# dronefreak/CABiNet

Hardware: AMD Instinct MI355X
Metric: 1024x1024 images/sec fwd+bwd (CABiNet-MobileNetV3-Large) (higher is better)
Workload: dtype f32; 1 GPU; BASELINE configs[2]: CABiNet-MobileNetV3-Large, 8x3x1024x1024 synthetic 8-class per GPU, fwd + 2x OhemCE + bwd + grad all-reduce + SGD step, HIP CAB/FFM kernels, fp32, random-init (model seed 0, gamma=0.5); per_gpu_batch=8, global_batch=8, n_classes=8, parallelism=dp1, miopen_find_mode=FAST

## Files before the change

### cabinet_amd/_lib.py

```python

from __future__ import annotations

import ctypes
import os
import threading

_PKG_DIR = os.path.dirname(os.path.abspath(__file__))
LIB_PATH = os.path.join(_PKG_DIR, "libcabinet_hip.so")
ABI_VERSION = 8

_c_float_p = ctypes.c_void_p
_INT, _FLT, _SZ, _PTR = ctypes.c_int, ctypes.c_float, ctypes.c_size_t, ctypes.c_void_p

SIGNATURES = {
    "cabinet_abi_version": (_INT, []),
    "cabinet_last_error": (ctypes.c_char_p, []),
    "cabinet_cab_attn_supported": (_INT, [_INT] * 2),
    "cabinet_cab_attn_precision_supported": (_INT, [_INT] * 3),
    "cabinet_cab_attn_fwd_workspace_bytes": (_SZ, [_INT] * 5),
    "cabinet_cab_attn_fwd": (_INT, [_PTR, _PTR, _PTR, _FLT, _INT, _INT, _INT, _INT, _INT, _PTR, _PTR, _PTR, _SZ, _PTR]),
    "cabinet_cab_attn_proj_supported": (_INT, [_INT] * 5),
    "cabinet_cab_attn_proj_fwd": (_INT, [_PTR] * 4 + [_FLT] + [_INT] * 5 + [_PTR] * 3 + [_PTR]),
    "cabinet_cab_attn_bwd_workspace_bytes": (_SZ, [_INT] * 4),
    "cabinet_cab_attn_bwd": (_INT, [_PTR] * 6 + [_FLT] + [_INT] * 4 + [_PTR] * 3 + [_PTR, _SZ, _PTR]),
# ... 22 lines not shown
    "cabinet_ohem_up_w_bwd_sel": (_INT, [_PTR] * 3 + [_INT] * 6 + [_PTR, _INT, _FLT] + [_PTR] + [_PTR, _SZ] + [_PTR, _PTR]),
    "cabinet_ohem_up_pair_w_bwd_sel": (_INT, [_PTR] * 4 + [_INT] * 6 + [_PTR, _INT, _FLT] + [_PTR] + [_PTR, _SZ] + [_PTR, _PTR, _PTR]),
    "cabinet_focal_up_supported": (_INT, [_INT] * 5 + [_FLT]),
    "cabinet_focal_up_fwd": (_INT, [_PTR] * 3 + [_INT] * 6 + [_FLT, _FLT, _INT] + [_PTR] * 3 + [_PTR, _PTR, _PTR]),
    "cabinet_focal_stats": (_INT, [_PTR, _PTR, _INT, _INT, _PTR, _PTR]),
    "cabinet_focal_up_bwd_workspace_bytes": (_SZ, [_INT] * 7),
    "cabinet_focal_up_bwd": (_INT, [_PTR] * 4 + [_INT] * 6 + [_FLT, _FLT, _INT, _FLT] + [_PTR] + [_PTR, _SZ] + [_PTR, _PTR, _PTR]),
    "cabinet_cab_qkv_supported": (_INT, [_INT] * 7 + [_PTR]),
    "cabinet_cab_qkv_padded_bins": (_INT, [_INT, _PTR]),
    "cabinet_cab_qkv_fwd_workspace_bytes": (_SZ, [_INT] * 7 + [_PTR]),
    "cabinet_cab_qkv_fwd": (_INT, [_PTR] * 14 + [_INT] * 7 + [_PTR] + [_INT, _FLT, _FLT] + [_PTR] * 10
                            + [_PTR, _SZ, _PTR]),
    "cabinet_cab_qkv_bwd_workspace_bytes": (_SZ, [_INT] * 7 + [_PTR]),
    "cabinet_cab_qkv_bwd": (_INT, [_PTR] * 20 + [_INT] * 7 + [_PTR] + [_INT] + [_PTR] * 9 + [_PTR, _SZ, _PTR]),
    "cabinet_conv1x1_fwd_workspace_bytes": (_SZ, [_INT] * 2),
    "cabinet_conv1x1_fwd": (_INT, [_PTR] * 2 + [_INT] * 4 + [_PTR] + [_PTR, _SZ, _PTR]),
    "cabinet_conv1x1_bias_supported": (_INT, [_INT] * 4),
    "cabinet_conv1x1_bias_fwd": (_INT, [_PTR] * 3 + [_INT] * 4 + [_PTR] + [_PTR, _SZ, _PTR]),
    "cabinet_channel_sum": (_INT, [_PTR] + [_INT] * 3 + [_PTR] + [_PTR]),
    "cabinet_conv1x1_bwd_workspace_bytes": (_SZ, [_INT] * 4),
    "cabinet_conv1x1_bwd": (_INT, [_PTR] * 3 + [_INT] * 4 + [_PTR] * 2 + [_PTR, _SZ, _PTR]),
    "cabinet_bn_act_workspace_bytes": (_SZ, [_INT] * 3),
    "cabinet_bn_act_fwd": (_INT, [_PTR] * 6 + [_INT] * 5 + [_FLT, _FLT] + [_PTR] * 3 + [_PTR, _SZ, _PTR]),
    "cabinet_bn_act_bwd": (_INT, [_PTR] * 6 + [_INT] * 5 + [_PTR] * 3 + [_PTR, _SZ, _PTR]),
    "cabinet_bn_cls_supported": (_INT, [_INT] * 3),
    "cabinet_bn_cls_table_floats": (_INT, [_INT] * 2),
    "cabinet_bn_cls_fwd_workspace_bytes": (_SZ, [_INT] * 3),
    "cabinet_bn_cls_fwd": (_INT, [_PTR] * 8 + [_INT] * 6 + [_FLT, _FLT] + [_PTR] * 2 + [_PTR, _SZ, _PTR]),
    "cabinet_bn_cls_bwd_workspace_bytes": (_SZ, [_INT] * 4),
    "cabinet_bn_cls_bwd": (_INT, [_PTR] * 3 + [_INT] * 6 + [_PTR] * 5 + [_PTR, _SZ, _PTR]),
    "cabinet_gate_act_fwd": (_INT, [_PTR] * 2 + [_INT] * 4 + [_PTR] + [_PTR]),
    "cabinet_gate_act_bwd_workspace_bytes": (_SZ, [_INT] * 3),
    "cabinet_gate_act_bwd": (_INT, [_PTR] * 3 + [_INT] * 4 + [_PTR] * 2 + [_PTR, _SZ, _PTR]),
    "cabinet_bn_dwconv_fwd_workspace_bytes": (_SZ, [_INT] * 4),
    "cabinet_bn_dwconv_fwd": (_INT, [_PTR] * 6 + [_INT] * 8 + [_FLT, _FLT] + [_PTR] * 3 + [_PTR, _SZ, _PTR]),
    "cabinet_bn_dwconv_bwd_workspace_bytes": (_SZ, [_INT] * 6),
    "cabinet_bn_dwconv_bwd": (_INT, [_PTR] * 7 + [_INT] * 8 + [_PTR] * 4 + [_PTR, _SZ, _PTR]),
    "cabinet_stem_conv_fwd": (_INT, [_PTR] * 2 + [_INT] * 3 + [_PTR] + [_PTR]),
    "cabinet_stem_conv_wrw_workspace_bytes": (_SZ, [_INT] * 3),
    "cabinet_stem_conv_wrw": (_INT, [_PTR] * 2 + [_INT] * 3 + [_PTR] + [_PTR, _SZ, _PTR]),
    "cabinet_stem_conv_bn_bwd_workspace_bytes": (_SZ, [_INT] * 3),
    "cabinet_stem_conv_bn_bwd": (_INT, [_PTR] * 7 + [_INT] * 4 + [_PTR] * 3 + [_PTR, _SZ, _PTR]),
    "cabinet_pwconv_supported": (_INT, [_INT] * 3),
    "cabinet_pwconv_fwd": (_INT, [_PTR] * 2 + [_INT] * 4 + [_PTR] + [_PTR]),
    "cabinet_pwconv_bwd_workspace_bytes": (_SZ, [_INT] * 4),
    "cabinet_pwconv_bwd": (_INT, [_PTR] * 3 + [_INT] * 4 + [_PTR] * 2 + [_PTR, _SZ, _PTR]),
    "cabinet_pwconv_wide_supported": (_INT, [_INT] * 3),
    "cabinet_pwconv_wide_wgrad_workspace_bytes": (_SZ, [_INT] * 4),
    "cabinet_pwconv_wide_wgrad": (_INT, [_PTR] * 2 + [_INT] * 4 + [_PTR] + [_PTR, _SZ, _PTR]),
    "cabinet_conv3x3s2_supported": (_INT, [_INT] * 2),
    "cabinet_conv3x3s2_wgrad_workspace_bytes": (_SZ, [_INT] * 5),
    "cabinet_conv3x3s2_wgrad": (_INT, [_PTR] * 2 + [_INT] * 5 + [_PTR] + [_PTR, _SZ, _PTR]),
    "cabinet_conv3x3s2_dgrad": (_INT, [_PTR] * 2 + [_INT] * 5 + [_PTR] + [_PTR]),
    "cabinet_bn_act_fwd_part": (_INT, [_PTR] * 7 + [_INT] * 6 + [_FLT, _FLT] + [_PTR] * 3 + [_PTR]),
    "cabinet_conv3x3_supported": (_INT, [_INT] * 3),
    "cabinet_conv3x3_tile_blocks": (_INT, [_INT] * 3),
    "cabinet_conv3x3_fwd_workspace_bytes": (_SZ, [_INT] * 6),
    "cabinet_conv3x3_fwd": (_INT, [_PTR] * 3 + [_INT] * 6 + [_PTR] * 2 + [_PTR, _SZ, _PTR]),
    "cabinet_conv3x3_bwd_workspace_bytes": (_SZ, [_INT] * 6),
    "cabinet_conv3x3_bwd": (_INT, [_PTR] * 4 + [_INT] * 6 + [_PTR] * 3 + [_PTR, _SZ, _PTR]),
    "cabinet_dwconv_supported": (_INT, [_INT] * 2),
    "cabinet_dwconv_fwd": (_INT, [_PTR] * 2 + [_INT] * 6 + [_PTR] + [_PTR]),
    "cabinet_dwconv_bwd_workspace_bytes": (_SZ, [_INT] * 6),
    "cabinet_dwconv_bwd": (_INT, [_PTR] * 3 + [_INT] * 6 + [_PTR] * 2 + [_PTR, _SZ, _PTR]),
    "cabinet_cab_local_supported": (_INT, [_INT] * 4),
    "cabinet_cab_local_fwd_workspace_bytes": (_SZ, [_INT] * 4),
    "cabinet_cab_local_bwd_workspace_bytes": (_SZ, [_INT] * 4),
    "cabinet_cab_local_fwd": (_INT, [_PTR] * 3 + [_PTR] * 5 + [_INT] * 5 + [_FLT, _FLT] + [_PTR] * 3 + [_PTR, _SZ, _PTR]),
    "cabinet_cab_local_bwd": (_INT, [_PTR] * 4 + [_PTR] * 3 + [_PTR] * 2 + [_INT] * 5 + [_PTR] * 3 + [_PTR] * 3 + [_PTR, _SZ, _PTR]),
    "cabinet_eval_chip_accum_supported": (_INT, [_INT] * 6),
    "cabinet_eval_chip_accum": (_INT, [_PTR] * 2 + [_INT] * 6 + [_PTR] + [_INT] * 4 + [_PTR] * 2 + [_PTR]),
    "cabinet_eval_scale_merge": (_INT, [_PTR] + [_INT] * 8 + [_PTR] + [_INT] * 2 + [_PTR]),
    "cabinet_eval_argmax_hist": (_INT, [_PTR] * 2 + [_INT] * 5 + [_PTR] * 2 + [_PTR]),
    "cabinet_predict_up_argmax_supported": (_INT, [_INT] * 5),
    "cabinet_predict_up_argmax": (_INT, [_PTR] + [_INT] * 6 + [_PTR] + [_PTR]),
    "cabinet_predict_argmax": (_INT, [_PTR] + [_INT] * 4 + [_PTR] + [_PTR]),
    "cabinet_predict_render": (_INT, [_PTR] * 3 + [_INT] + [_PTR] * 2 + [_FLT] + [_INT] * 3 + [_PTR] * 3 + [_PTR]),
    "cabinet_se_act_bwd_workspace_bytes": (_SZ, [_INT] * 3),
    "cabinet_se_act_bwd_reduce": (_INT, [_PTR] * 8 + [_INT] * 4 + [_PTR] * 2 + [_PTR, _SZ, _PTR]),
    "cabinet_se_act_bwd_coef": (_INT, [_PTR] * 3 + [_INT] * 4 + [_PTR] * 4 + [_PTR]),
    "cabinet_se_act_bwd_dx": (_INT, [_PTR] * 9 + [_INT] * 4 + [_PTR] + [_PTR]),
    "cabinet_sgd_tail_workspace_bytes": (_SZ, [_INT]),
    "cabinet_sgd_tail_state_bytes": (_SZ, [_INT]),
    "cabinet_sgd_tail_step": (_INT, [_PTR, _INT, _PTR, _INT, _PTR, _PTR, _SZ, _INT, _PTR, _SZ, _PTR]),
    "cabinet_grad_accum_state_bytes": (_SZ, []),
    "cabinet_grad_accum": (_INT, [_PTR, _INT, _PTR, _INT, _PTR, _SZ, _INT, _PTR]),
    "cabinet_grad_accum_reset": (_INT, [_PTR, _SZ, _PTR]),
    "cabinet_augment_supported": (_INT, [_INT] * 7),
    "cabinet_augment_workspace_bytes": (_SZ, [_INT] * 3),
    "cabinet_augment_batch": (_INT, [_PTR] + [_INT] * 3 + [_PTR, ctypes.c_ulonglong] + [_PTR] * 5 + [_PTR, _SZ, _PTR]),
    "cabinet_augment_warp_supported": (_INT, [_INT] * 4 + [ctypes.c_double] * 2),
    "cabinet_augment_warp_batch": (_INT, [_PTR] + [_INT] * 3 + [_PTR]),
    "cabinet_augment_resize_batch": (_INT, [_PTR] + [_INT] * 3 + [_PTR]),
}

_lock = threading.Lock()
_lib = None


def _preload_hip_runtime():
    import sys

    cands = []
    if "torch" in sys.modules:
        cands.append(os.path.join(os.path.dirname(sys.modules["torch"].__file__), "lib", "libamdhip64.so"))
    cands += ["libamdhip64.so.7", "/opt/rocm/lib/libamdhip64.so.7"]
# ... 44 lines not shown
```

### cabinet_amd/csrc/capi.hip

```cpp
#include "../../include/cabinet_hip.h"

#include <stdarg.h>
#include <stdint.h>
#include <stdio.h>

#include "blocks.hpp"
#include "cab_local.hpp"
#include "cab_qkv.hpp"
#include "common.hpp"

namespace cabinet {
int attn_fwd_kvsplit(int B, int n);
bool attn_shape_supported(int Kc, int Vc);
hipError_t attn_fwd_dispatch(const float* q, const float* k, const float* v, float scale, int B, int Kc,
                             int Vc, int n, float* ctx, float* lse, float* part_ctx, float* part_lse,
                             int kvsplit, hipStream_t stream);
bool attn_fwd_proj_supported(int B, int Kc, int Vc, int Co, int n);
hipError_t attn_fwd_proj_dispatch(const float* q, const float* k, const float* v, const float* w_out, float scale, int B, int Kc,
                                  int Vc, int Co, int n, float* ctx, float* glob, float* lse, hipStream_t stream);
bool attn_bf16_supported(int Kc, int Vc);
size_t attn_bf16_pack_bytes(int B, int Kc, int Vc, int n, int precision);
hipError_t attn_fwd_bf16_dispatch(const float* q, const float* k, const float* v, float scale, int B, int Kc, int Vc, int n,
                                  float* ctx, float* lse, float* part_ctx, float* part_lse, int kvsplit, void* pack, int precision,
                                  hipStream_t stream);
// ... 49 lines not shown
hipError_t se_act_bwd_coef_run(const float* sums, const float* gate, const float* ds, int B, int C, int P, int training,
                               float* dweight, float* dbias, float* coef, float* ds_p, hipStream_t stream);
hipError_t se_act_bwd_dx_run(const float* dy, const float* z, const float* mean, const float* invstd, const float* weight,
                             const float* bias, const float* gate, const float* ds_p, const float* coef, int B, int C, int P,
                             int act, float* dz, hipStream_t stream);
size_t gate_act_workspace(int rows, int P);
hipError_t gate_act_fwd_run(const float* x, const float* gate, int rows, int P, int act, float* y, hipStream_t stream);
hipError_t gate_act_bwd_run(const float* dy, const float* x, const float* gate, int rows, int P, int act, float* dx,
                            float* dgate, void* ws, hipStream_t stream);
bool bn_cls_supported(int C, int K, int P);
int bn_cls_table_floats(int C, int K);
size_t bn_cls_fwd_workspace(int B, int C, int P);
size_t bn_cls_bwd_workspace(int B, int C, int K, int P);
hipError_t bn_cls_fwd_run(const float* z, const float* conv_part, const float* bn_w, const float* bn_b, float* run_mean, float* run_var,
                          const float* w_cls, const float* bias, int B, int C, int K, int H, int W, int training, float momentum,
                          float eps, float* y, float* tab, void* ws, hipStream_t stream);
hipError_t bn_cls_bwd_run(const float* dy, const float* z, const float* tab, int B, int C, int K, int H, int W, int training, float* dz,
                          float* dbn_w, float* dbn_b, float* dw_cls, float* dbias, void* ws, hipStream_t stream);
bool dwconv_supported(int K, int S);
size_t dwconv_bwd_workspace(int B, int C, int H, int W, int K);
hipError_t dwconv_fwd_run(const float* x, const float* w, int B, int C, int H, int W, int K, int S, float* y,
                          hipStream_t stream);
hipError_t dwconv_bwd_run(const float* dy, const float* x, const float* w, int B, int C, int H, int W, int K, int S,
                          float* dx, float* dw, void* ws, hipStream_t stream);
size_t bn_dwconv_fwd_workspace(int B, int C, int H, int W);
size_t bn_dwconv_bwd_workspace(int B, int C, int H, int W, int K);
hipError_t bn_dwconv_fwd_run(const float* z, const float* bn_w, const float* bn_b, float* run_mean, float* run_var,
                             const float* w, int B, int C, int H, int W, int K, int S, int act, int training,
                             float momentum, float eps, float* y, float* save_mean, float* save_invstd, void* ws,
                             hipStream_t stream);
hipError_t bn_dwconv_bwd_run(const float* dy, const float* z, const float* bn_w, const float* bn_b,
                             const float* save_mean, const float* save_invstd, const float* w, int B, int C, int H,
                             int W, int K, int S, int act, int training, float* dz, float* dbn_w, float* dbn_b,
                             float* dw, void* ws, hipStream_t stream);
size_t stem_conv_wrw_workspace(int B, int H, int W);
hipError_t stem_conv_fwd_run(const float* x, const float* w, int B, int H, int W, float* y, hipStream_t stream);
size_t stem_conv_bn_bwd_workspace(int B, int H, int W);
hipError_t stem_conv_bn_bwd_run(const float* g, const float* z, const float* x, const float* bn_weight, const float* bn_bias,
                                const float* save_mean, const float* save_invstd, int B, int H, int W, int training, float* dw,
                                float* dbn_weight, float* dbn_bias, void* ws, hipStream_t stream);
hipError_t stem_conv_wrw_run(const float* dy, const float* x, int B, int H, int W, float* dw, void* ws,
                             hipStream_t stream);
bool pwconv_wide_supported(int Ci, int Co, int P);
size_t pwconv_wide_wgrad_workspace(int B, int Ci, int Co, int P);
hipError_t pwconv_wide_wgrad_run(const float* dy, const float* x, int B, int Ci, int Co, int P, float* dw, void* ws,
                                 hipStream_t stream);
bool conv3x3s2_supported(int Ci, int Co);
long long conv3x3s2_wgrad_slabs(int B, int Ci, int H, int W);
size_t conv3x3s2_wgrad_workspace(int B, int Ci, int H, int W);
hipError_t conv3x3s2_wgrad_run(const float* dy, const float* x, int B, int Ci, int H, int W, float* dw, void* ws,
                               hipStream_t stream);
long long conv3x3s2_dgrad_workgroups(int B, int H, int W);
hipError_t conv3x3s2_dgrad_run(const float* dy, const float* w, int B, int H, int W, float* dx, hipStream_t stream);
bool pwconv_supported(int Ci, int Co, int P);
size_t pwconv_bwd_workspace(int B, int Ci, int Co, int P);
hipError_t pwconv_fwd_run(const float* x, const float* w, int B, int Ci, int Co, int P, float* y, hipStream_t stream);
hipError_t pwconv_bwd_run(const float* dy, const float* x, const float* w, int B, int Ci, int Co, int P, float* dx,
                          float* dw, void* ws, hipStream_t stream);
int ohem_blocks(int B, int H, int W);
hipError_t ohem_up_fwd_run(int nh, const float* const* low, const long long* labels, int B, int C, int Hl, int Wl, int H, int W,
                           float thresh, int ignore_lb, float* const* loss_px, float* const* blk_sum, int* const* blk_cnt,
                           const float* const* class_weight, hipStream_t stream, const float* focal_gamma = nullptr);
hipError_t focal_stats_run(const float* blk_sum, const int* blk_cnt, int nheads, int nblk, double* stats, hipStream_t stream);
hipError_t ohem_stats_run(const float* blk_sum, const int* blk_cnt, int nheads, int nblk, double* stats, hipStream_t stream);
size_t ohem_up_bwd_workspace(int B, int C, int H, int Wl);
bool ohem_up_supported(int C, int Wl, int W);
hipError_t ohem_up_bwd_run(int nh, const float* const* low, const long long* labels, const float* const* loss_px, int B, int C,
                           int Hl, int Wl, int H, int W, float thresh, int ignore_lb, float coef, float* dlow, void* ws,
                           const float* const* cw, const double* dsel, hipStream_t stream, const float* focal_gamma = nullptr);
size_t ohem_select_workspace(int nheads);
hipError_t ohem_select_run(int nheads, const float* const* loss_px, const long long* labels, const double* stats, long long P, int C,
                           float thresh, const int* n_min, int ignore_lb, const float* const* cw, double* sel, void* ws,
                           hipStream_t stream);
struct WinoShape {
    int B, C0, C1, K, H, W;
};
bool conv3x3_supported(int C0, int C1, int K);
bool conv3x3_shape_ok(const WinoShape& s);
int conv3x3_tile_blocks(int B, int H, int W);
size_t conv3x3_fwd_workspace(const WinoShape& s);
size_t conv3x3_bwd_workspace(const WinoShape& s);
hipError_t conv3x3_fwd_run(const WinoShape& s, const float* x0, const float* x1, const float* w, float* y, float* stat_part, void* ws,
                           hipStream_t stream);
hipError_t conv3x3_bwd_run(const WinoShape& s, const float* dy, const float* x0, const float* x1, const float* w, float* dx0,
                           float* dx1, float* dw, void* ws, hipStream_t stream);
int eval_chip_threads(int C, int wl, int cw, int nsrc);
hipError_t eval_chip_accum_run(const float* a, const float* b, int N, int C, int hl, int wl, int ch, int cw, float* dst, int FH,
                               int FW, int y0, int x0, const float* rcp_y, const float* rcp_x, hipStream_t stream);
hipError_t eval_scale_merge_run(const float* prob, int N, int C, int FH, int FW, int hst, int hed, int wst, int wed, float* total,
                                int H, int W, hipStream_t stream);
hipError_t eval_argmax_hist_run(const float* total, const long long* labels, int N, int C, int H, int W, int ignore_lb, long long* hist,
                                unsigned char* pred, hipStream_t stream);
int predict_up_threads(int C, int wl, int W);
hipError_t predict_up_argmax_run(const float* a, int N, int C, int hl, int wl, int H, int W, unsigned char* labels, hipStream_t stream);
hipError_t predict_argmax_run(const float* total, int N, int C, int H, int W, unsigned char* labels, hipStream_t stream);
hipError_t predict_render_run(const unsigned char* labels, const float* image, const unsigned char* palette, int n_colors,
                              const float* mean, const float* std, float alpha, int N, int H, int W, unsigned char* pred,
                              unsigned char* inp, unsigned char* ovl, hipStream_t stream);
hipError_t augment_warp_run(const void* descs, int N, int max_oh, int max_ow, hipStream_t stream);
hipError_t augment_resize_run(const void* descs, int N, int max_oh, int max_ow, hipStream_t stream);
size_t augment_workspace(int N, int th, int tw);
hipError_t augment_run(const void* samples, int N, int th, int tw, const float* noise, unsigned long long seed, const float* mean,
                       const float* std, float* out_image, long long* out_label, unsigned char* out_u8, void* workspace,
                       hipStream_t stream);
size_t sgd_tail_workspace(int n_chunks);
size_t sgd_tail_state(int n_entries);
// ... 1115 lines not shown
        return fail(CABINET_ERR_UNSUPPORTED, "pwconv_wide_wgrad: B=%d, P=%d: more than 2^30 pixel chunks", B, P);
    if (!cabinet::pwconv_wide_supported(Ci, Co, P))
        return fail(CABINET_ERR_UNSUPPORTED, "pwconv_wide_wgrad: Ci=%d, Co=%d, P=%d (multiples of 8, <= 4096, P <= 2^21, max(Ci, Co) * P <= 2^28)",
                    Ci, Co, P);
    if (!dy || !x || !dw) return fail(CABINET_ERR_INVALID_ARG, "pwconv_wide_wgrad: null tensor pointer");
    const size_t need = cabinet::pwconv_wide_wgrad_workspace(B, Ci, Co, P);
    if (!workspace || workspace_bytes < need)
        return fail(CABINET_ERR_WORKSPACE, "pwconv_wide_wgrad: workspace %zu < %zu bytes", workspace_bytes, need);
    return hip_status(cabinet::pwconv_wide_wgrad_run(dy, x, B, Ci, Co, P, dw, workspace, static_cast<hipStream_t>(stream)),
                      "pwconv_wide_wgrad launch");
}

static bool conv3x3s2_size_ok(int B, int Ci, int H, int W) {
    return cabinet::conv3x3s2_wgrad_slabs(B, Ci, H, W) <= (1ll << 30);
}

int cabinet_conv3x3s2_supported(int Ci, int Co) { return cabinet::conv3x3s2_supported(Ci, Co) ? 1 : 0; }

size_t cabinet_conv3x3s2_wgrad_workspace_bytes(int B, int Ci, int Co, int H, int W) {
    if (B <= 0 || H <= 0 || W <= 0 || !cabinet::conv3x3s2_supported(Ci, Co) || !conv3x3s2_size_ok(B, Ci, H, W)) return 0;
    return cabinet::conv3x3s2_wgrad_workspace(B, Ci, H, W);
}

int cabinet_conv3x3s2_wgrad(const float* dy, const float* x, int B, int Ci, int Co, int H, int W, float* dw, void* workspace,
                            size_t workspace_bytes, cabinet_stream_t stream) {
    if (B <= 0 || Ci <= 0 || Co <= 0 || H <= 0 || W <= 0)
        return fail(CABINET_ERR_INVALID_ARG, "conv3x3s2_wgrad: non-positive dimension");
    if (!cabinet::conv3x3s2_supported(Ci, Co))
        return fail(CABINET_ERR_UNSUPPORTED, "conv3x3s2_wgrad: Ci=%d, Co=%d ((64, 64) and (3, 16) are compiled)", Ci, Co);
    if (!conv3x3s2_size_ok(B, Ci, H, W))
        return fail(CABINET_ERR_UNSUPPORTED, "conv3x3s2_wgrad: B=%d, H=%d, W=%d: grid too large", B, H, W);
    if (!dy || !x || !dw) return fail(CABINET_ERR_INVALID_ARG, "conv3x3s2_wgrad: null tensor pointer");
    const size_t need = cabinet::conv3x3s2_wgrad_workspace(B, Ci, H, W);
    if (!workspace || workspace_bytes < need)
        return fail(CABINET_ERR_WORKSPACE, "conv3x3s2_wgrad: workspace %zu < %zu bytes", workspace_bytes, need);
    return hip_status(cabinet::conv3x3s2_wgrad_run(dy, x, B, Ci, H, W, dw, workspace, static_cast<hipStream_t>(stream)),
                      "conv3x3s2_wgrad launch");
}

int cabinet_conv3x3s2_dgrad(const float* dy, const float* w, int B, int Ci, int Co, int H, int W, float* dx,
                            cabinet_stream_t stream) {
    if (B <= 0 || Ci <= 0 || Co <= 0 || H <= 0 || W <= 0)
        return fail(CABINET_ERR_INVALID_ARG, "conv3x3s2_dgrad: non-positive dimension");
    if (Ci != 64 || Co != 64)
        return fail(CABINET_ERR_UNSUPPORTED, "conv3x3s2_dgrad: Ci=%d, Co=%d ((64, 64) is compiled)", Ci, Co);
    if (cabinet::conv3x3s2_dgrad_workgroups(B, H, W) > (1ll << 30))
        return fail(CABINET_ERR_UNSUPPORTED, "conv3x3s2_dgrad: B=%d, H=%d, W=%d: grid too large", B, H, W);
    if (!dy || !w || !dx) return fail(CABINET_ERR_INVALID_ARG, "conv3x3s2_dgrad: null tensor pointer");
    if ((reinterpret_cast<size_t>(dx) & 7) != 0)
        return fail(CABINET_ERR_INVALID_ARG, "conv3x3s2_dgrad: dx must be 8-byte aligned");
    return hip_status(cabinet::conv3x3s2_dgrad_run(dy, w, B, H, W, dx, static_cast<hipStream_t>(stream)), "conv3x3s2_dgrad launch");
}

static int check_conv3x3(const cabinet::WinoShape& s, const char* who) {
    if (s.B <= 0 || s.C0 <= 0 || s.C1 < 0 || s.K <= 0 || s.H <= 0 || s.W <= 0)
        return fail(CABINET_ERR_INVALID_ARG, "%s: non-positive dimension", who);
    if (!cabinet::conv3x3_shape_ok(s))
        return fail(CABINET_ERR_UNSUPPORTED,
                    "%s: C0=%d C1=%d Co=%d H=%d W=%d (C0, C1 multiples of 16; Co, C0+C1 multiples of 64; C0 %% 64 == 0 when C1 > 0; "
                    "one image's tensors < 1 GiB)", who, s.C0, s.C1, s.K, s.H, s.W);
    return CABINET_OK;
}

int cabinet_conv3x3_supported(int C0, int C1, int Co) { return cabinet::conv3x3_supported(C0, C1, Co) ? 1 : 0; }

int cabinet_conv3x3_tile_blocks(int B, int H, int W) {
    return B > 0 && H > 0 && W > 0 ? cabinet::conv3x3_tile_blocks(B, H, W) : 0;
}

size_t cabinet_conv3x3_fwd_workspace_bytes(int B, int C0, int C1, int Co, int H, int W) {
    const cabinet::WinoShape s{B, C0, C1, Co, H, W};
    return B > 0 && H > 0 && W > 0 && cabinet::conv3x3_shape_ok(s) ? cabinet::conv3x3_fwd_workspace(s) : 0;
}

int cabinet_conv3x3_fwd(const float* x0, const float* x1, const float* w, int B, int C0, int C1, int Co, int H, int W, float* y,
                        float* bn_part, void* workspace, size_t workspace_bytes, cabinet_stream_t stream) {
    const cabinet::WinoShape s{B, C0, C1, Co, H, W};
    if (int rc = check_conv3x3(s, "conv3x3_fwd")) return rc;
    if (!x0 || !w || !y || (C1 > 0 && !x1)) return fail(CABINET_ERR_INVALID_ARG, "conv3x3_fwd: null tensor pointer");
    CABINET_REQUIRE_ALIGNED("conv3x3_fwd", x0, x1, w, y, bn_part);
    const size_t need = cabinet::conv3x3_fwd_workspace(s);
    if (!workspace || workspace_bytes < need)
        return fail(CABINET_ERR_WORKSPACE, "conv3x3_fwd: workspace %zu < %zu bytes", workspace_bytes, need);
    return hip_status(cabinet::conv3x3_fwd_run(s, x0, C1 > 0 ? x1 : nullptr, w, y, bn_part, workspace, static_cast<hipStream_t>(stream)),
                      "conv3x3_fwd launch");
}

size_t cabinet_conv3x3_bwd_workspace_bytes(int B, int C0, int C1, int Co, int H, int W) {
    const cabinet::WinoShape s{B, C0, C1, Co, H, W};
    return B > 0 && H > 0 && W > 0 && cabinet::conv3x3_shape_ok(s) ? cabinet::conv3x3_bwd_workspace(s) : 0;
}

int cabinet_conv3x3_bwd(const float* dy, const float* x0, const float* x1, const float* w, int B, int C0, int C1, int Co, int H,
                        int W, float* dx0, float* dx1, float* dw, void* workspace, size_t workspace_bytes, cabinet_stream_t stream) {
    const cabinet::WinoShape s{B, C0, C1, Co, H, W};
    if (int rc = check_conv3x3(s, "conv3x3_bwd")) return rc;
    if (!dy || !w || (dw && (!x0 || (C1 > 0 && !x1))) || (dx0 && C1 > 0 && !dx1))
        return fail(CABINET_ERR_INVALID_ARG, "conv3x3_bwd: null tensor pointer");
    CABINET_REQUIRE_ALIGNED("conv3x3_bwd", dy, x0, x1, w, dx0, dx1, dw);
    const size_t need = cabinet::conv3x3_bwd_workspace(s);
    if (!workspace || workspace_bytes < need)
        return fail(CABINET_ERR_WORKSPACE, "conv3x3_bwd: workspace %zu < %zu bytes", workspace_bytes, need);
    return hip_status(cabinet::conv3x3_bwd_run(s, dy, x0, C1 > 0 ? x1 : nullptr, w, dx0, C1 > 0 ? dx1 : nullptr, dw, workspace,
                                               static_cast<hipStream_t>(stream)),
                      "conv3x3_bwd launch");
}
// ... 209 lines not shown
```

### cabinet_amd/csrc/conv3x3_s2.hip

```cpp
#include "common.hpp"
#include "slab_sum.hpp"

namespace cabinet {

struct C3Shape {
    int B, H, W, Ho, Wo;
};

static C3Shape c3_shape(int B, int H, int W) { return C3Shape{B, H, W, (H - 1) / 2 + 1, (W - 1) / 2 + 1}; }

constexpr int CW_C = 64;
constexpr int CW_TW = 32;
constexpr int CW_IW = 2 * CW_TW + 1;
constexpr int CW_XP = 3 * CW_IW;
constexpr int CW_DLD = CW_TW + 1;
constexpr int CW_SLAB = CW_C * CW_C * 9;
constexpr int CW_TARGET_WG = 512;
constexpr int CW_MIN_ROWS = 4;

struct C3Plan {
    int tiles_x, strips, rows_per;
};

static C3Plan cw_plan(const C3Shape& s) {
// ... 236 lines not shown
        const float* bp0 = brow + s0 * CD_RP;
        const float* bp1 = brow + s1 * CD_RP;
        s0 = s1;
#pragma unroll 1
        for (int ng = 0; ng < CD_NT / 16 && n0 + 16 * ng < s.Wo; ++ng) {
            f32x4v acc[2][2];
#pragma unroll
            for (int i = 0; i < 2; ++i)
#pragma unroll
                for (int j = 0; j < 2; ++j) acc[i][j] = f32x4v{0.f, 0.f, 0.f, 0.f};
            float bv[2][8];
            auto read_half = [&](int g, float* v) {
                const int t = g / 2;
                const float* bt = (cd_shift(t / 3) ? bp1 : bp0) + 16 * ng + cd_shift(t % 3);
#pragma unroll
                for (int i = 0; i < 8; ++i) v[i] = bt[4 * (8 * (g % 2) + i) * CD_CP];
            };
            read_half(0, bv[0]);
            f32x4v p0, p1;
#pragma unroll
            for (int g = 0; g < 18; ++g) {
                const int t = g / 2, k8 = 8 * (g % 2);
                if (g + 1 < 18) read_half(g + 1, bv[(g + 1) & 1]);
                if (g % 2 == 0) p0 = p1 = f32x4v{0.f, 0.f, 0.f, 0.f};
#pragma unroll
                for (int i = 0; i < 8; i += 2) {
                    p0 = mfma16(wr[t][k8 + i], bv[g & 1][i], p0);
                    p1 = mfma16(wr[t][k8 + i + 1], bv[g & 1][i + 1], p1);
                }
                if (g % 2 == 1) acc[cd_par(t / 3)][cd_par(t % 3)] += p0 + p1;
                __builtin_amdgcn_sched_barrier(0);
            }
            const int ix = 2 * (n0 + 16 * ng + lc);
#pragma unroll
            for (int rp = 0; rp < 2; ++rp) {
                const int iy = 2 * m + rp;
                if (iy < s.H && ix < s.W) {
#pragma unroll
                    for (int r = 0; r < 4; ++r) {
                        float* p = dxb + ((size_t)r * s.H + iy) * s.W + ix;
                        if (pair_ok) {
                            *reinterpret_cast<f32x2*>(p) = f32x2{acc[rp][0][r], acc[rp][1][r]};
                        } else {
                            p[0] = acc[rp][0][r];
                            if (ix + 1 < s.W) p[1] = acc[rp][1][r];
                        }
                    }
                }
            }
        }
    }
}

bool conv3x3s2_supported(int Ci, int Co) { return (Ci == CW_C && Co == CW_C) || (Ci == CF_CI && Co == CF_CO); }

static C3Plan cd_plan(const C3Shape& s) {
    C3Plan p;
    p.tiles_x = ceil_div(s.Wo, CD_NT);
    const long per = (long)s.B * p.tiles_x;
    long strips = CW_TARGET_WG / per;
    if (strips > s.Ho) strips = s.Ho;
    if (strips < 1) strips = 1;
    p.rows_per = ceil_div(s.Ho, (int)strips);
    p.strips = ceil_div(s.Ho, p.rows_per);
    return p;
}

long long conv3x3s2_dgrad_workgroups(int B, int H, int W) {
    const C3Shape s = c3_shape(B, H, W);
    const long long per = (long long)B * ceil_div(s.Wo, CD_NT);
    if (per > (1ll << 30)) return per;
    const C3Plan p = cd_plan(s);
    return per * p.strips;
}

hipError_t conv3x3s2_dgrad_run(const float* dy, const float* w, int B, int H, int W, float* dx, hipStream_t stream) {
    const C3Shape s = c3_shape(B, H, W);
    const C3Plan p = cd_plan(s);
    hipLaunchKernelGGL(conv3x3s2_dgrad64_kernel, dim3(B * p.tiles_x * p.strips), dim3(256), 0, stream, dy, w, s, p.tiles_x,
                       p.strips, p.rows_per, dx);
    return hipGetLastError();
}

long long conv3x3s2_wgrad_slabs(int B, int Ci, int H, int W) {
    const C3Shape s = c3_shape(B, H, W);
    if (Ci == CF_CI) return (long long)B * ceil_div(s.Ho, CF_TH);
    const long long tiles_x = ceil_div(s.Wo, CW_TW);
    if ((long long)B * tiles_x > (1ll << 30)) return (long long)B * tiles_x;
    const C3Plan p = cw_plan(s);
    return (long long)B * p.tiles_x * p.strips;
}

size_t conv3x3s2_wgrad_workspace(int B, int Ci, int H, int W) {
    return align_up((size_t)conv3x3s2_wgrad_slabs(B, Ci, H, W) * (Ci == CF_CI ? CF_SLAB : CW_SLAB) * sizeof(float), 256);
}

hipError_t conv3x3s2_wgrad_run(const float* dy, const float* x, int B, int Ci, int H, int W, float* dw, void* ws,
                               hipStream_t stream) {
    const C3Shape s = c3_shape(B, H, W);
    float* slabs = static_cast<float*>(ws);
    const int nslab = (int)conv3x3s2_wgrad_slabs(B, Ci, H, W);
    if (Ci == CF_CI) {
        hipLaunchKernelGGL(conv3x3s2_wgrad_3_16_kernel, dim3(nslab), dim3(256), 0, stream, dy, x, s, ceil_div(s.Wo, CF_TW),
                           slabs);
    } else {
        const C3Plan p = cw_plan(s);
        const size_t lds = (size_t)(CW_C * CW_XP + CW_C * CW_DLD) * sizeof(float);
// ... 14 lines not shown
```

### cabinet_amd/functional.py

```python

from __future__ import annotations

import ctypes as _ct

import torch
import torch.nn.functional as F

from . import _lib


def _ptr(t):
    return t.data_ptr() if t is not None else None


def _stream_handle(device):
    return torch.cuda.current_stream(device).cuda_stream


def _workspace(nbytes, device):
    if nbytes == 0:
        return None, 0
    ws = torch.empty(nbytes, dtype=torch.uint8, device=device)
    return ws, nbytes

# ... 1626 lines not shown
                                                   _stream_handle(x.device))
            _lib.check(rc, "cabinet_pwconv_wide_wgrad")
        return dx, dw


def pwconv_wide(x, conv):
    if not x.is_cuda:
        raise RuntimeError("pwconv_wide: device tensors only")
    return _PwConvWide.apply(x, conv.weight)




CONV3X3S2_ENABLED = _os.environ.get("CABINET_CONV3X3S2", "1") != "0"


def conv3x3s2_supported(conv, x):
    if not (CONV3X3S2_ENABLED and isinstance(conv, torch.nn.Conv2d) and x.is_cuda and x.dim() == 4):
        return False
    if not (conv.kernel_size == (3, 3) and conv.stride == (2, 2) and conv.padding == (1, 1) and conv.groups == 1
            and conv.bias is None and conv.dilation == (1, 1) and conv.padding_mode == "zeros"):
        return False
    if not (torch.is_grad_enabled() and conv.weight.requires_grad) or torch.is_autocast_enabled():
        return False
    if x.dtype != torch.float32 or conv.weight.dtype != torch.float32 or x.shape[0] < 1 or x.shape[2] * x.shape[3] < 1:
        return False
    return x.shape[1] == conv.in_channels and bool(_lib.load().cabinet_conv3x3s2_supported(conv.in_channels, conv.out_channels))


def _conv3x3s2_native_wgrad(Ci, B, H):
    return Ci == 3 and B * (((H - 1) // 2 + 1 + 3) // 4) >= 1024


CONV3X3S2_WGRAD64_ENABLED = _os.environ.get("CABINET_CONV3X3S2_WGRAD64", "1") != "0"
_CW_MIN_WORKGROUPS = 256
_CW_MIN_ROWS = 4


def _conv3x3s2_wgrad64_plan(B, H, W):
    Ho, Wo = (H - 1) // 2 + 1, (W - 1) // 2 + 1
    tiles = -(-Wo // 32)
    strips = max(1, min(512 // (B * tiles), -(-Ho // 4)))
    rows_per = -(-Ho // strips)
    return B * tiles * -(-Ho // rows_per), rows_per


def _conv3x3s2_native_wgrad64(B, H, W):
    if not CONV3X3S2_WGRAD64_ENABLED:
        return False
    workgroups, rows_per = _conv3x3s2_wgrad64_plan(B, H, W)
    return workgroups >= _CW_MIN_WORKGROUPS and rows_per >= _CW_MIN_ROWS


class _Conv3x3S2(torch.autograd.Function):

    @staticmethod
    def forward(fn_ctx, x, weight):
        x = x.contiguous()
        y = F.conv2d(x, weight, None, 2, 1)
        fn_ctx.save_for_backward(x, weight)
        return y

    @staticmethod
    def backward(fn_ctx, g):
        x, w = fn_ctx.saved_tensors
        g = g.contiguous()
        lib = _lib.load()
        xc, gc = _f32c(x), _f32c(g)
        Co, Ci = w.shape[0], w.shape[1]
        B, H, W = xc.shape[0], xc.shape[2], xc.shape[3]
        cb = torch.ops.aten.convolution_backward
        dx = None
        if fn_ctx.needs_input_grad[0] and Ci == 64:
            dx = torch.empty_like(xc)
            with torch.cuda.device(x.device):
                rc = lib.cabinet_conv3x3s2_dgrad(_ptr(gc), _ptr(_f32c(w)), B, Ci, Co, H, W, _ptr(dx), _stream_handle(x.device))
            _lib.check(rc, "cabinet_conv3x3s2_dgrad")
        elif fn_ctx.needs_input_grad[0]:
            dx = cb(g, x, w, None, [2, 2], [1, 1], [1, 1], False, [0, 0], 1, [True, False, False])[0]
        dw = None
        native_dw = _conv3x3s2_native_wgrad64(B, H, W) if Ci == 64 else _conv3x3s2_native_wgrad(Ci, B, H)
        if fn_ctx.needs_input_grad[1] and native_dw:
            dw = torch.empty((Co, Ci, 3, 3), dtype=torch.float32, device=x.device)
            ws, nbytes = _workspace(lib.cabinet_conv3x3s2_wgrad_workspace_bytes(B, Ci, Co, H, W), x.device)
            with torch.cuda.device(x.device):
                rc = lib.cabinet_conv3x3s2_wgrad(_ptr(gc), _ptr(xc), B, Ci, Co, H, W, _ptr(dw), _ptr(ws), nbytes,
                                                 _stream_handle(x.device))
            _lib.check(rc, "cabinet_conv3x3s2_wgrad")
        elif fn_ctx.needs_input_grad[1]:
            dw = cb(g, x, w, None, [2, 2], [1, 1], [1, 1], False, [0, 0], 1, [False, True, False])[1]
        return dx, dw


class Conv2dS2(torch.nn.Conv2d):

    def _conv_forward(self, input, weight, bias):
        if bias is None and conv3x3s2_supported(self, input):
            return _Conv3x3S2.apply(input, weight)
        return super()._conv_forward(input, weight, bias)




def eval_chip_accum_supported(logits, chip_size, flip=False):
    if not (logits.is_cuda and logits.dim() == 4 and _lib.available()):
        return False
    _, C, hl, wl = logits.shape
    return bool(_lib.load().cabinet_eval_chip_accum_supported(C, hl, wl, int(chip_size[0]), int(chip_size[1]), int(bool(flip))))


def eval_chip_accum(dst, logits, logits_flipped, chip_size, origin, rcp_y=None, rcp_x=None):
    lib = _lib.load()
    if not (dst.is_cuda and dst.dtype == torch.float32 and dst.is_contiguous()):
        raise RuntimeError("eval_chip_accum: dst must be a dense fp32 device tensor")
    a = _f32c(logits)
    b = _f32c(logits_flipped) if logits_flipped is not None else None
    if b is not None and b.shape != a.shape:
        raise RuntimeError("eval_chip_accum: the flipped chip's logits must have the shape of the chip's")
    N, C, hl, wl = a.shape
    if dst.shape[:2] != (N, C):
        raise RuntimeError(f"eval_chip_accum: dst {tuple(dst.shape)} does not match logits {tuple(a.shape)}")
    FH, FW = dst.shape[2:]
    ry = _f32c(rcp_y) if rcp_y is not None else None
    rx = _f32c(rcp_x) if rcp_x is not None else None
    if (ry is not None and ry.numel() != FH) or (rx is not None and rx.numel() != FW):
        raise RuntimeError("eval_chip_accum: rcp_y / rcp_x must have one entry per row / column of dst")
    dev = dst.device
    with torch.cuda.device(dev):
        rc = lib.cabinet_eval_chip_accum(_ptr(a), _ptr(b), N, C, hl, wl, int(chip_size[0]), int(chip_size[1]), _ptr(dst), FH, FW,
                                         int(origin[0]), int(origin[1]), _ptr(ry), _ptr(rx), _stream_handle(dev))
    _lib.check(rc, "cabinet_eval_chip_accum")
    return dst


def eval_scale_merge_supported(total):
    return bool(total.is_cuda and total.dim() == 4 and _lib.available() and total.shape[0] * total.shape[1] <= 65535
                and total.shape[2] <= 65535)


def eval_scale_merge(total, prob, crop=None):
    lib = _lib.load()
    if not (total.is_cuda and total.dtype == torch.float32 and total.is_contiguous()):
        raise RuntimeError("eval_scale_merge: total must be a dense fp32 device tensor")
    prob = _f32c(prob)
    N, C, H, W = total.shape
    if prob.shape[:2] != (N, C):
        raise RuntimeError(f"eval_scale_merge: prob {tuple(prob.shape)} does not match total {tuple(total.shape)}")
    FH, FW = prob.shape[2:]
    hst, hed, wst, wed = crop if crop is not None else (0, FH, 0, FW)
    dev = total.device
    with torch.cuda.device(dev):
# ... 110 lines not shown
```

### include/cabinet_hip.h

```cpp
#ifndef CABINET_HIP_H_
#define CABINET_HIP_H_

#include <stddef.h>

#ifdef __cplusplus
extern "C" {
#endif

#define CABINET_ABI_VERSION 8

#define CABINET_OK 0
#define CABINET_ERR_INVALID_ARG (-1)
#define CABINET_ERR_UNSUPPORTED (-2)
#define CABINET_ERR_WORKSPACE (-3)
#define CABINET_ERR_HIP (-4)

typedef void* cabinet_stream_t;

int cabinet_abi_version(void);
const char* cabinet_last_error(void);

#define CABINET_PREC_FP32 0
#define CABINET_PREC_BF16X3 1
#define CABINET_PREC_BF16X6 2
// ... 244 lines not shown
size_t cabinet_stem_conv_wrw_workspace_bytes(int B, int H, int W);
int cabinet_stem_conv_wrw(const float* dy, const float* x, int B, int H, int W, float* dw,
                          void* workspace, size_t workspace_bytes, cabinet_stream_t stream);

size_t cabinet_stem_conv_bn_bwd_workspace_bytes(int B, int H, int W);
int cabinet_stem_conv_bn_bwd(const float* g, const float* z, const float* x, const float* bn_weight, const float* bn_bias,
                             const float* save_mean, const float* save_invstd, int B, int H, int W, int training,
                             float* dw, float* dbn_weight, float* dbn_bias,
                             void* workspace, size_t workspace_bytes, cabinet_stream_t stream);

int cabinet_pwconv_supported(int Ci, int Co, int P);
int cabinet_pwconv_fwd(const float* x, const float* w, int B, int Ci, int Co, int P, float* y, cabinet_stream_t stream);
size_t cabinet_pwconv_bwd_workspace_bytes(int B, int Ci, int Co, int P);
int cabinet_pwconv_bwd(const float* dy, const float* x, const float* w, int B, int Ci, int Co, int P,
                       float* dx, float* dw, void* workspace, size_t workspace_bytes, cabinet_stream_t stream);

int cabinet_pwconv_wide_supported(int Ci, int Co, int P);
size_t cabinet_pwconv_wide_wgrad_workspace_bytes(int B, int Ci, int Co, int P);
int cabinet_pwconv_wide_wgrad(const float* dy, const float* x, int B, int Ci, int Co, int P, float* dw,
                              void* workspace, size_t workspace_bytes, cabinet_stream_t stream);

int cabinet_conv3x3_supported(int C0, int C1, int Co);
int cabinet_conv3x3_tile_blocks(int B, int H, int W);
size_t cabinet_conv3x3_fwd_workspace_bytes(int B, int C0, int C1, int Co, int H, int W);
int cabinet_conv3x3_fwd(const float* x0, const float* x1, const float* w, int B, int C0, int C1, int Co, int H, int W,
                        float* y, float* bn_part, void* workspace, size_t workspace_bytes, cabinet_stream_t stream);
size_t cabinet_conv3x3_bwd_workspace_bytes(int B, int C0, int C1, int Co, int H, int W);
int cabinet_conv3x3_bwd(const float* dy, const float* x0, const float* x1, const float* w, int B, int C0, int C1, int Co,
                        int H, int W, float* dx0, float* dx1, float* dw,
                        void* workspace, size_t workspace_bytes, cabinet_stream_t stream);

int cabinet_eval_chip_accum_supported(int C, int hl, int wl, int ch, int cw, int flip);
int cabinet_eval_chip_accum(const float* a, const float* b, int N, int C, int hl, int wl, int ch, int cw, float* dst, int FH, int FW,
                            int y0, int x0, const float* rcp_y, const float* rcp_x, cabinet_stream_t stream);
int cabinet_eval_scale_merge(const float* prob, int N, int C, int FH, int FW, int hst, int hed, int wst, int wed, float* total, int H,
                             int W, cabinet_stream_t stream);
int cabinet_eval_argmax_hist(const float* total, const long long* labels, int N, int C, int H, int W, int ignore_lb, long long* hist,
                             unsigned char* pred, cabinet_stream_t stream);

int cabinet_predict_up_argmax_supported(int C, int hl, int wl, int H, int W);
int cabinet_predict_up_argmax(const float* logits_low, int N, int C, int hl, int wl, int H, int W, unsigned char* labels,
                              cabinet_stream_t stream);
int cabinet_predict_argmax(const float* total, int N, int C, int H, int W, unsigned char* labels, cabinet_stream_t stream);
int cabinet_predict_render(const unsigned char* labels, const float* image, const unsigned char* palette, int n_colors,
                           const float* mean, const float* std, float alpha, int N, int H, int W, unsigned char* pred_rgb,
                           unsigned char* input_rgb, unsigned char* overlay_rgb, cabinet_stream_t stream);

int cabinet_conv3x3s2_supported(int Ci, int Co);
size_t cabinet_conv3x3s2_wgrad_workspace_bytes(int B, int Ci, int Co, int H, int W);
int cabinet_conv3x3s2_wgrad(const float* dy, const float* x, int B, int Ci, int Co, int H, int W, float* dw,
                            void* workspace, size_t workspace_bytes, cabinet_stream_t stream);
int cabinet_conv3x3s2_dgrad(const float* dy, const float* w, int B, int Ci, int Co, int H, int W, float* dx,
                            cabinet_stream_t stream);

#define CABINET_SGD_TAIL_CHUNK 4096
#define CABINET_SGD_TAIL_EMA_ONLY 1

typedef struct cabinet_sgd_tail_entry {
    float* param;
    const float* grad;
    float* buf;
    float* ema;
    long long numel;
    int group;
    int flags;
} cabinet_sgd_tail_entry;

typedef struct cabinet_sgd_tail_chunk {
    long long start;
    int tensor;
    int length;
} cabinet_sgd_tail_chunk;

typedef struct cabinet_sgd_tail_config {
    double lr0, warmup_start_lr, max_iter, power;
    double lr_scale[4], weight_decay[4];
    double momentum, max_norm, ema_decay, ema_tau;
    long long warmup_steps;
    int skip_nonfinite;
    int reserved;
} cabinet_sgd_tail_config;

size_t cabinet_sgd_tail_workspace_bytes(int n_chunks);
size_t cabinet_sgd_tail_state_bytes(int n_entries);
int cabinet_sgd_tail_step(const cabinet_sgd_tail_entry* entries, int n_entries, const cabinet_sgd_tail_chunk* chunks, int n_chunks,
                          const cabinet_sgd_tail_config* config, void* state, size_t state_bytes, int max_grid,
                          void* workspace, size_t workspace_bytes, cabinet_stream_t stream);

typedef struct cabinet_grad_accum_entry {
    float* acc;
    const float* grad;
    long long numel;
} cabinet_grad_accum_entry;

size_t cabinet_grad_accum_state_bytes(void);
int cabinet_grad_accum(const cabinet_grad_accum_entry* entries, int n_entries, const cabinet_sgd_tail_chunk* chunks, int n_chunks,
                       void* state, size_t state_bytes, int max_grid, cabinet_stream_t stream);
int cabinet_grad_accum_reset(void* state, size_t state_bytes, cabinet_stream_t stream);

#define CABINET_AUGMENT_GRAY 1
#define CABINET_AUGMENT_GAMMA 2
#define CABINET_AUGMENT_NOISE 4
#define CABINET_AUGMENT_CUTOUT 8

typedef struct cabinet_augment_tap {
    int first, step, n;
// ... 53 lines not shown
```

Before: 394.2 images/s.

## Add native MFMA forward kernel for 64-channel stride-2 3x3 conv

Result: faster. 400.3 images/s (median of 6 runs) (+1.5%).

```diff
diff --git a/cabinet_amd/_lib.py b/cabinet_amd/_lib.py
--- a/cabinet_amd/_lib.py
+++ b/cabinet_amd/_lib.py
@@ -98,6 +98,8 @@
     "cabinet_conv3x3s2_wgrad_workspace_bytes": (_SZ, [_INT] * 5),
     "cabinet_conv3x3s2_wgrad": (_INT, [_PTR] * 2 + [_INT] * 5 + [_PTR] + [_PTR, _SZ, _PTR]),
     "cabinet_conv3x3s2_dgrad": (_INT, [_PTR] * 2 + [_INT] * 5 + [_PTR] + [_PTR]),
+    "cabinet_conv3x3s2_fwd_supported": (_INT, [_INT] * 2),
+    "cabinet_conv3x3s2_fwd": (_INT, [_PTR] * 2 + [_INT] * 5 + [_PTR] + [_PTR]),
     "cabinet_bn_act_fwd_part": (_INT, [_PTR] * 7 + [_INT] * 6 + [_FLT, _FLT] + [_PTR] * 3 + [_PTR]),
     "cabinet_conv3x3_supported": (_INT, [_INT] * 3),
     "cabinet_conv3x3_tile_blocks": (_INT, [_INT] * 3),
diff --git a/cabinet_amd/csrc/capi.hip b/cabinet_amd/csrc/capi.hip
--- a/cabinet_amd/csrc/capi.hip
+++ b/cabinet_amd/csrc/capi.hip
@@ -125,6 +125,9 @@
                                hipStream_t stream);
 long long conv3x3s2_dgrad_workgroups(int B, int H, int W);
 hipError_t conv3x3s2_dgrad_run(const float* dy, const float* w, int B, int H, int W, float* dx, hipStream_t stream);
+bool conv3x3s2_fwd_supported(int Ci, int Co);
+long long conv3x3s2_fwd_workgroups(int B, int H, int W);
+hipError_t conv3x3s2_fwd_run(const float* x, const float* w, int B, int H, int W, float* y, hipStream_t stream);
 bool pwconv_supported(int Ci, int Co, int P);
 size_t pwconv_bwd_workspace(int B, int Ci, int Co, int P);
 hipError_t pwconv_fwd_run(const float* x, const float* w, int B, int Ci, int Co, int P, float* y, hipStream_t stream);
@@ -1346,6 +1349,19 @@
     return hip_status(cabinet::conv3x3s2_dgrad_run(dy, w, B, H, W, dx, static_cast<hipStream_t>(stream)), "conv3x3s2_dgrad launch");
 }
 
+int cabinet_conv3x3s2_fwd_supported(int Ci, int Co) { return cabinet::conv3x3s2_fwd_supported(Ci, Co) ? 1 : 0; }
+
+int cabinet_conv3x3s2_fwd(const float* x, const float* w, int B, int Ci, int Co, int H, int W, float* y, cabinet_stream_t stream) {
+    if (B <= 0 || Ci <= 0 || Co <= 0 || H <= 0 || W <= 0)
+        return fail(CABINET_ERR_INVALID_ARG, "conv3x3s2_fwd: non-positive dimension");
+    if (!cabinet::conv3x3s2_fwd_supported(Ci, Co))
+        return fail(CABINET_ERR_UNSUPPORTED, "conv3x3s2_fwd: Ci=%d, Co=%d ((64, 64) is compiled)", Ci, Co);
+    if (cabinet::conv3x3s2_fwd_workgroups(B, H, W) > (1ll << 30))
+        return fail(CABINET_ERR_UNSUPPORTED, "conv3x3s2_fwd: B=%d, H=%d, W=%d: grid too large", B, H, W);
+    if (!x || !w || !y) return fail(CABINET_ERR_INVALID_ARG, "conv3x3s2_fwd: null tensor pointer");
+    return hip_status(cabinet::conv3x3s2_fwd_run(x, w, B, H, W, y, static_cast<hipStream_t>(stream)), "conv3x3s2_fwd launch");
+}
+
 static int check_conv3x3(const cabinet::WinoShape& s, const char* who) {
     if (s.B <= 0 || s.C0 <= 0 || s.C1 < 0 || s.K <= 0 || s.H <= 0 || s.W <= 0)
         return fail(CABINET_ERR_INVALID_ARG, "%s: non-positive dimension", who);
diff --git a/cabinet_amd/csrc/conv3x3_s2.hip b/cabinet_amd/csrc/conv3x3_s2.hip
--- a/cabinet_amd/csrc/conv3x3_s2.hip
+++ b/cabinet_amd/csrc/conv3x3_s2.hip
@@ -312,7 +312,183 @@
     }
 }
 
+#ifndef CABINET_CV_TW
+#define CABINET_CV_TW 32
+#endif
+constexpr int CV_TW = CABINET_CV_TW;
+constexpr int CV_NSEG = CV_TW / 32;
+constexpr int CV_EV = 0;
+constexpr int CV_OD = CV_TW + 1;
+constexpr int CV_RP = 2 * CV_TW + 2;
+constexpr int CV_CP = (3 * CV_RP - 16 + 31) / 32 * 32 + 16;
+constexpr int CV_PR = CW_C / 4;
+constexpr int CV_WG_PER_CU = CV_TW == 32 ? 2 : 1;
+constexpr int CV_TARGET_WG = 256 * CV_WG_PER_CU;
+constexpr size_t CV_LDS = (size_t)CW_C * CV_CP * sizeof(float);
+static_assert(CV_TW == 32 || CV_TW == 64, "the staging covers a row with one or two 64-lane segments");
+static_assert(CV_CP % 32 == 16 && CV_CP >= 3 * CV_RP, "k-groups lk and lk + 1 of a 32-lane read group on disjoint banks");
+
+__host__ __device__ constexpr int cv_koff(int kx) { return kx == 0 ? CV_EV : kx == 1 ? CV_OD : CV_EV + 1; }
+
+__global__ __launch_bounds__(256, CV_WG_PER_CU) void conv3x3s2_fwd64_kernel(const float* __restrict__ x, const float* __restrict__ w,
+                                                                          C3Shape s, int tiles_x, int strips, int rows_per,
+                                                                          float* __restrict__ y) {
+    extern __shared__ __attribute__((aligned(16))) float smem[];
+    float* xs = smem;
+    const int tid = threadIdx.x, wave = __builtin_amdgcn_readfirstlane(tid >> 6), lane = tid & 63, lc = lane & 15, lk = lane >> 4;
+    int bi = blockIdx.x;
+    const int tx = bi % tiles_x;
+    bi /= tiles_x;
+    const int strip = bi % strips, b = bi / strips;
+    const int oy_begin = strip * rows_per, oy_end = min(s.Ho, oy_begin + rows_per);
+    const int ox0 = tx * CV_TW, ix0 = 2 * ox0 - 1;
+    const int co0 = 16 * wave;
+
+    float wr[9][16];
+#pragma unroll
+    for (int t = 0; t < 9; ++t)
+#pragma unroll
+        for (int ks = 0; ks < 16; ++ks) wr[t][ks] = w[((co0 + lc) * CW_C + 4 * ks + lk) * 9 + t];
+
+    const float* xb = x + (size_t)b * CW_C * s.H * s.W;
+    float* yb = y + ((size_t)b * CW_C + co0 + 4 * lk) * s.Ho * s.Wo;
+    const float* brow = xs + lk * CV_CP + lc;
+    unsigned colo[CV_NSEG];
+    int dcol[CV_NSEG];
+    bool col_ok[CV_NSEG];
+#pragma unroll
+    for (int sg = 0; sg < CV_NSEG; ++sg) {
+        const int c = 64 * sg + lane;
+        colo[sg] = (unsigned)min(2 * ox0 + c, s.W - 1) * 4u;
+        col_ok[sg] = 2 * ox0 + c < s.W;
+        dcol[sg] = (c & 1) ? CV_EV + (c + 1) / 2 : CV_OD + c / 2;
+    }
+    const bool halo_ok = ix0 >= 0;
+    const int hrow = tid >> 6, hch = tid & 63;
+    float xr[2 * CV_PR * CV_NSEG], xh;
+    auto request = [&](int nr, int iya, int iyb) {
+        const int ya = min(max(iya, 0), s.H - 1), yb_ = min(max(iyb, 0), s.H - 1);
+#pragma unroll
+        for (int j = 0; j < CV_PR; ++j)
+#pragma unroll
+            for (int sg = 0; sg < CV_NSEG; ++sg)
+                xr[j * CV_NSEG + sg] = cd_ld(xb + ((size_t)(CV_PR * wave + j) * s.H + ya) * s.W, colo[sg]);
+        if (nr == 2) {
+#pragma unroll
+            for (int j = 0; j < CV_PR; ++j)
+#pragma unroll
+                for (int sg = 0; sg < CV_NSEG; ++sg)
+                    xr[(CV_PR + j) * CV_NSEG + sg] = cd_ld(xb + ((size_t)(CV_PR * wave + j) * s.H + yb_) * s.W, colo[sg]);
+        }
+        xh = xb[((size_t)hch * s.H + (hrow == 0 ? ya : yb_)) * s.W + max(ix0, 0)];
+    };
+    auto commit = [&](int nr, int iya, int iyb, int sa, int sb) {
+        const bool oka = iya >= 0 && iya < s.H, okb = iyb >= 0 && iyb < s.H;
+        float* d = xs + CV_PR * wave * CV_CP;
+#pragma unroll
+        for (int j = 0; j < CV_PR; ++j)
+#pragma unroll
+            for (int sg = 0; sg < CV_NSEG; ++sg)
+                d[j * CV_CP + sa * CV_RP + dcol[sg]] = (oka && col_ok[sg]) ? xr[j * CV_NSEG + sg] : 0.f;
+        if (nr == 2) {
+#pragma unroll
+            for (int j = 0; j < CV_PR; ++j)
+#pragma unroll
+                for (int sg = 0; sg < CV_NSEG; ++sg)
+                    d[j * CV_CP + sb * CV_RP + dcol[sg]] = (okb && col_ok[sg]) ? xr[(CV_PR + j) * CV_NSEG + sg] : 0.f;
+        }
+        if (hrow < nr) xs[hch * CV_CP + (hrow == 0 ? sa : sb) * CV_RP + CV_EV] = ((hrow == 0 ? oka : okb) && halo_ok) ? xh : 0.f;
+    };
+    const int iy_begin = 2 * oy_begin - 1;
+    request(2, iy_begin, iy_begin + 1);
+    commit(2, iy_begin, iy_begin + 1, 0, 1);
+    request(1, iy_begin + 2, iy_begin + 2);
+    commit(1, iy_begin + 2, iy_begin + 2, 2, 2);
+    __syncthreads();
+    int s0 = 0;
+    for (int oy = oy_begin; oy < oy_end; ++oy) {
+        const int s1 = s0 == 2 ? 0 : s0 + 1, s2 = s1 == 2 ? 0 : s1 + 1;
+        const bool more = oy + 1 < oy_end;
+        if (more) request(2, 2 * oy + 2, 2 * oy + 3);
+        const float* bp0 = brow + s0 * CV_RP;
+        const float* bp1 = brow + s1 * CV_RP;
+        const float* bp2 = brow + s2 * CV_RP;
+#pragma unroll 1
+        for (int ng = 0; ng < CV_TW / 16 && ox0 + 16 * ng < s.Wo; ++ng) {
+            f32x4v acc = f32x4v{0.f, 0.f, 0.f, 0.f};
+            float bv[2][8];
+            auto read_half = [&](int g, float* v) {
+                const int t = g / 2, ky = t / 3;
+                const float* bt = (ky == 0 ? bp0 : ky == 1 ? bp1 : bp2) + 16 * ng + cv_koff(t % 3);
+#pragma unroll
+                for (int i = 0; i < 8; ++i) v[i] = bt[4 * (8 * (g % 2) + i) * CV_CP];
+            };
+            read_half(0, bv[0]);
+            f32x4v p0, p1;
+#pragma unroll
+            for (int g = 0; g < 18; ++g) {
+                const int t = g / 2, k8 = 8 * (g % 2);
+                if (g + 1 < 18) read_half(g + 1, bv[(g + 1) & 1]);
+                if (g % 2 == 0) p0 = p1 = f32x4v{0.f, 0.f, 0.f, 0.f};
+#pragma unroll
+                for (int i = 0; i < 8; i += 2) {
+                    p0 = mfma16(wr[t][k8 + i], bv[g & 1][i], p0);
+                    p1 = mfma16(wr[t][k8 + i + 1], bv[g & 1][i + 1], p1);
+                }
+                if (g % 2 == 1) {
+                    acc += p0 + p1;
+                    asm volatile("" : "+v"(acc));
+                }
+                __builtin_amdgcn_sched_barrier(0);
+            }
+            const int ox = ox0 + 16 * ng + lc;
+            if (ox < s.Wo) {
+#pragma unroll
+                for (int r = 0; r < 4; ++r) yb[((size_t)r * s.Ho + oy) * s.Wo + ox] = acc[r];
+            }
+        }
+        if (more) {
+            __syncthreads();
+            commit(2, 2 * oy + 2, 2 * oy + 3, s0, s1);
+            __syncthreads();
+        }
+        s0 = s2;
+    }
+}
+
 bool conv3x3s2_supported(int Ci, int Co) { return (Ci == CW_C && Co == CW_C) || (Ci == CF_CI && Co == CF_CO); }
+bool conv3x3s2_fwd_supported(int Ci, int Co) { return Ci == CW_C && Co == CW_C; }
+
+static C3Plan cv_plan(const C3Shape& s) {
+    C3Plan p;
+    p.tiles_x = ceil_div(s.Wo, CV_TW);
+    const long per = (long)s.B * p.tiles_x;
+    long strips = CV_TARGET_WG / per;
+    if (strips > s.Ho) strips = s.Ho;
+    if (strips < 1) strips = 1;
+    p.rows_per = ceil_div(s.Ho, (int)strips);
+    p.strips = ceil_div(s.Ho, p.rows_per);
+    return p;
+}
+
+long long conv3x3s2_fwd_workgroups(int B, int H, int W) {
+    const C3Shape s = c3_shape(B, H, W);
+    const long long per = (long long)B * ceil_div(s.Wo, CV_TW);
+    if (per > (1ll << 30)) return per;
+    const C3Plan p = cv_plan(s);
+    return per * p.strips;
+}
+
+hipError_t conv3x3s2_fwd_run(const float* x, const float* w, int B, int H, int W, float* y, hipStream_t stream) {
+    const C3Shape s = c3_shape(B, H, W);
+    const C3Plan p = cv_plan(s);
+    static lds_attr_mask mask{0};
+    if (hipError_t e = ensure_dynamic_lds(reinterpret_cast<const void*>(conv3x3s2_fwd64_kernel), CV_LDS, mask); e != hipSuccess)
+        return e;
+    hipLaunchKernelGGL(conv3x3s2_fwd64_kernel, dim3(B * p.tiles_x * p.strips), dim3(256), CV_LDS, stream, x, w, s, p.tiles_x,
+                       p.strips, p.rows_per, y);
+    return hipGetLastError();
+}
 
 static C3Plan cd_plan(const C3Shape& s) {
     C3Plan p;
diff --git a/cabinet_amd/functional.py b/cabinet_amd/functional.py
--- a/cabinet_amd/functional.py
+++ b/cabinet_amd/functional.py
@@ -1702,12 +1702,65 @@
     return workgroups >= _CW_MIN_WORKGROUPS and rows_per >= _CW_MIN_ROWS
 
 
+CONV3X3S2_FWD64_ENABLED = _os.environ.get("CABINET_CONV3X3S2_FWD64", "1") != "0"
+_CV_TILE = 32
+_CV_MIN_WORKGROUPS = 256
+_CV_MIN_ROWS = 2
+
+
+def _conv3x3s2_fwd64_plan(B, H, W):
+    Ho, Wo = (H - 1) // 2 + 1, (W - 1) // 2 + 1
+    tiles = -(-Wo // _CV_TILE)
+    strips = max(1, min(512 // (B * tiles), Ho))
+    rows_per = -(-Ho // strips)
+    return B * tiles * -(-Ho // rows_per), rows_per
+
+
+def _conv3x3s2_native_fwd64(B, H, W):
+    if not CONV3X3S2_FWD64_ENABLED:
+        return False
+    workgroups, rows_per = _conv3x3s2_fwd64_plan(B, H, W)
+    return workgroups >= _CV_MIN_WORKGROUPS and rows_per >= _CV_MIN_ROWS
+
+
+def conv3x3s2_fwd64(x, weight):
+    if not (x.is_cuda and x.dim() == 4 and x.dtype == torch.float32 and weight.dtype == torch.float32
+            and tuple(weight.shape) == (64, 64, 3, 3) and x.shape[1] == 64):
+        raise RuntimeError("conv3x3s2_fwd64: fp32 device tensors, x (B, 64, H, W), weight (64, 64, 3, 3)")
+    xc, wc = _f32c(x.detach()), _f32c(weight.detach())
+    B, H, W = xc.shape[0], xc.shape[2], xc.shape[3]
+    y = torch.empty((B, 64, (H - 1) // 2 + 1, (W - 1) // 2 + 1), dtype=torch.float32, device=x.device)
+    with torch.cuda.device(x.device):
+        rc = _lib.load().cabinet_conv3x3s2_fwd(_ptr(xc), _ptr(wc), B, 64, 64, H, W, _ptr(y), _stream_handle(x.device))
+    _lib.check(rc, "cabinet_conv3x3s2_fwd")
+    return y
+
+
+def _conv3x3s2_fwd64_nograd(conv, x, weight):
+    if not (CONV3X3S2_ENABLED and x.is_cuda and x.dim() == 4 and x.shape[0] >= 1 and x.shape[2] * x.shape[3] >= 1):
+        return False
+    if not (conv.kernel_size == (3, 3) and conv.stride == (2, 2) and conv.padding == (1, 1) and conv.groups == 1
+            and conv.bias is None and conv.dilation == (1, 1) and conv.padding_mode == "zeros"
+            and conv.in_channels == 64 and conv.out_channels == 64 and x.shape[1] == 64):
+        return False
+    if torch.is_autocast_enabled() or x.dtype != torch.float32 or weight.dtype != torch.float32 or not weight.is_cuda:
+        return False
+    if torch.is_grad_enabled() and (x.requires_grad or weight.requires_grad):
+        return False
+    if not _conv3x3s2_native_fwd64(x.shape[0], x.shape[2], x.shape[3]):
+        return False
+    return bool(_lib.load().cabinet_conv3x3s2_fwd_supported(64, 64))
+
+
 class _Conv3x3S2(torch.autograd.Function):
 
     @staticmethod
     def forward(fn_ctx, x, weight):
         x = x.contiguous()
-        y = F.conv2d(x, weight, None, 2, 1)
+        if weight.shape[0] == 64 and weight.shape[1] == 64 and _conv3x3s2_native_fwd64(x.shape[0], x.shape[2], x.shape[3]):
+            y = conv3x3s2_fwd64(x, weight)
+        else:
+            y = F.conv2d(x, weight, None, 2, 1)
         fn_ctx.save_for_backward(x, weight)
         return y
 
@@ -1747,6 +1800,8 @@
     def _conv_forward(self, input, weight, bias):
         if bias is None and conv3x3s2_supported(self, input):
             return _Conv3x3S2.apply(input, weight)
+        if bias is None and _conv3x3s2_fwd64_nograd(self, input, weight):
+            return conv3x3s2_fwd64(input, weight)
         return super()._conv_forward(input, weight, bias)
 
 
diff --git a/include/cabinet_hip.h b/include/cabinet_hip.h
--- a/include/cabinet_hip.h
+++ b/include/cabinet_hip.h
@@ -320,6 +320,9 @@
                             void* workspace, size_t workspace_bytes, cabinet_stream_t stream);
 int cabinet_conv3x3s2_dgrad(const float* dy, const float* w, int B, int Ci, int Co, int H, int W, float* dx,
                             cabinet_stream_t stream);
+int cabinet_conv3x3s2_fwd_supported(int Ci, int Co);
+int cabinet_conv3x3s2_fwd(const float* x, const float* w, int B, int Ci, int Co, int H, int W, float* y,
+                          cabinet_stream_t stream);
 
 #define CABINET_SGD_TAIL_CHUNK 4096
 #define CABINET_SGD_TAIL_EMA_ONLY 1
```
